# lmangani/duckdb-fastlane

Measured on AMD Instinct MI355X. Metric: decoded values/sec (lineitem_full SF100 full scan), higher is better.
Workload: dtype u8..u64 integer unpack -> int32/int64/string_t

## Files before the change

### duckdb-fastlane_amd/csrc/fls_decode.hpp

```cpp
#pragma once
#include <hip/hip_runtime.h>

#include <cstdint>
#include <vector>

namespace fls {

struct DevChunk {
    const uint8_t *chunk;
    const uint8_t *dict;
    uint8_t *out;
    uint32_t nvec;
    uint32_t dict_count;
    uint32_t meta_off;
    uint32_t packed_off;
    uint32_t aux_off;
    uint8_t enc, T, vbits, ob;
    uint64_t heap_host;
    uint32_t heap_bytes;
    union {
        uint32_t vec_base;
        uint32_t max_w;
    };
};
static_assert(sizeof(DevChunk) == 64, "DevChunk is 64 B");

enum : uint32_t { KERR_DICT_CODE = 1, KERR_RUN_INDEX = 2, KERR_BAD_DESC = 4, KERR_FSST = 8 };
enum : uint32_t { KERR_LDS_BASE = 32 };

struct DecodeGeom {
    uint32_t p_bytes = 256, v_bytes = 0;
    int grid = 0;
};

struct SplitPlan {
    uint32_t waves = 0, pieces = 0;
    bool guided = false;
    size_t positions() const { return waves ? (size_t)waves + pieces + 2 : 0; }
};

hipError_t launch_decode(const DevChunk *d_chunks, uint32_t nchunks, uint32_t *d_err, const DecodeGeom &geom,
                         hipStream_t stream, uint32_t *d_queue = nullptr, const uint32_t *d_split = nullptr,
                         SplitPlan plan = SplitPlan(), bool shared_queue = false, int prio = 0);
uint32_t decode_waves(const DecodeGeom &geom);
SplitPlan balanced_split(const DevChunk *h, uint32_t n, uint32_t nw, uint32_t static_pct, uint32_t pieces_per_wave,
                         std::vector<uint32_t> &pos);
SplitPlan guided_split(const DevChunk *h, uint32_t n, uint32_t nw, uint32_t factor, uint32_t min_vecs,
                       std::vector<uint32_t> &pos);
enum : int {
    kFsstPlain = 1, kFsstTwoQ = 2, kFsstZeroFlush = 4, kFsstW6 = 8, kFsstCirc = 16, kFsstLenFromSym = 32, kFsstAbsLds = 64, kFsstEarlyGather = 128,
    kFsstDefault = kFsstW6 | kFsstZeroFlush | kFsstAbsLds,
    kFsstSegSparse = kFsstPlain,
    kFsstSegPackedLen = kFsstLenFromSym,
    kFsstSegWide = kFsstCirc,
    kFsstSegDouble = kFsstEarlyGather,
    kFsstSegBatch = 256,
    kFsstAblateRecords = 512, kFsstAblateFlush = 1024, kFsstAblateWrite = 2048,
    kFsstSegLean = 4096,
    kFsstSegD8 = 8192,
    kFsstSegLazy = 16384,
    kFsstSegW4 = 32768
};
struct FsstLaunch {
    int bytes_per_lane = 8;
    bool small = false;
    uint32_t *queue = nullptr;
    bool reset_queue = true;
    int waves_per_cu = 0;
    int grid_cus = 0;
    int variant = kFsstDefault;
    bool seg = false;
    int seg_cap = 4096;
};
hipError_t launch_fsst(const DevChunk *d_chunks, uint32_t nchunks, uint32_t nvecs, uint32_t *d_err,
                       hipStream_t stream, const FsstLaunch &how);
struct FusedLaunch {
    uint32_t fsst_per16 = 6;
    uint32_t piece = 2;
    bool halving = false;
    uint32_t fsst_static_pct = 0;
    bool static_first = true;
    int waves_per_cu = 0;
    int x = 0;
    uint32_t tail_chunks = 0, tail_split = 1;
};
hipError_t launch_fused(const DevChunk *d_main, uint32_t nmain, const DevChunk *d_fsst, uint32_t nfsst,
                        uint32_t nfvecs, bool small, uint32_t *d_err, const DecodeGeom &geom, hipStream_t stream,
                        uint32_t *d_queues, const FusedLaunch &how);
bool fsst_variant_built(int variant, bool seg, int bytes_per_lane);
bool fused_x_built(int x);
hipError_t launch_fsst_sp(const DevChunk *d_chunks, uint32_t nchunks, uint32_t nvecs, uint32_t *d_err,
                          hipStream_t stream);
int decode_grid_size(uint32_t shmem_per_block);
int device_cus();
int occupancy(const void *kernel, int block, size_t shmem);

bool &rating_launch();

struct ProbeRegion {
    uint8_t *out;
    uint64_t bytes;
};
hipError_t probe_placement(const ProbeRegion *d_regions, uint32_t nregions, uint8_t *const *bufs,
                           const uint64_t *buf_bytes, uint32_t nbuf, int reps, hipStream_t stream, float *chunk_ms,
                           float *fill_ms);
inline void chunk_lds_need(uint8_t enc, uint8_t T, uint8_t ob, uint32_t dict_count, uint32_t max_w,
                           uint32_t &p_bytes, uint32_t &v_bytes) {
    p_bytes = 128 * max_w + 128;
    v_bytes = 0;
    if (enc == 2  && T < 64) v_bytes = 128 * T;
    if (enc == 4 ) v_bytes = 2048;
    if (enc == 3 ) {
        const uint32_t d = dict_count * ob;
        v_bytes = 4096 + (d <= 4096 ? ((d + 15) & ~15u) : 0);
    }
}

}
```

### duckdb-fastlane_amd/csrc/flsgpu.hip

```cpp
#include <fcntl.h>
#include <hip/hip_runtime.h>
#include <hip/hip_ext.h>
#include <sys/mman.h>
#include <sys/stat.h>
#include <unistd.h>

#include <algorithm>
#include <atomic>
#include <condition_variable>
#include <cstring>
#include <map>
#include <mutex>
#include <memory>
#include <string>
#include <chrono>
#include <cmath>
#include <thread>
#include <vector>

#include "../../include/flsgpu.h"
#include "fls_agg.hpp"
#include "fls_common.hpp"
#include "fls_config.hpp"
#include "fls_decode.hpp"
// ... 459 lines not shown
                }
        }
        auto d = std::make_unique<ScanDev>();
        d->dev = dev;
        return d;
    }
    void give(std::unique_ptr<ScanDev> d) {
        if (!d) return;
        d->sync();
        if (d->free_batches.size() != d->batches.size()) return;
        for (auto &sl : d->slots) {
            sl.busy = sl.starved = false;
            sl.hb = nullptr;
        }
        d->free_batches.clear();
        for (auto &b : d->batches) d->free_batches.push_back(b.get());
        std::lock_guard<std::mutex> lk(mu);
        size_t same = 0;
        for (auto &x : idle) same += x->dev == d->dev;
        if (same >= kIdlePerDev) return;
        const int dev = d->dev;
        idle.push_back(std::move(d));
        trim_locked(dev, idle_cap_bytes());
    }
    size_t idle_pinned() {
        std::lock_guard<std::mutex> lk(mu);
        size_t t = 0;
        for (auto &d : idle) t += pinned_bytes(*d);
        return t;
    }
};

}

struct fls_connection {
    std::vector<int> devices;
    std::shared_ptr<ConnRes> res = std::make_shared<ConnRes>();
};

struct SideStream {
    hipStream_t stream = nullptr;
    hipEvent_t fork = nullptr, join = nullptr;
    int cu_m = 0;
    hipStream_t cu_a = nullptr, cu_b = nullptr;
    hipEvent_t join_a = nullptr, join_b = nullptr;
    void release_cu() {
        for (hipStream_t *st : {&cu_a, &cu_b})
            if (*st) {
                hipStreamSynchronize(*st);
                hipStreamDestroy(*st);
                *st = nullptr;
            }
        for (hipEvent_t *e : {&join_a, &join_b})
            if (*e) {
                hipEventDestroy(*e);
                *e = nullptr;
            }
        cu_m = 0;
    }
};

namespace {

struct Resident {
    int dev = -1;
    uint32_t rg0 = 0, rg1 = 0;
    uint64_t base = 0;
    uint64_t first_row = 0, rows = 0;
    DevBuf<uint8_t> img;
    DevBuf<StrT> strtab;
    std::vector<uint64_t> strtab_off;
    DevBuf<uint32_t> err;
    DevBuf<uint32_t> queue;
    std::vector<DevBuf<uint8_t>> d_heap;
    std::vector<PinBuf<uint8_t>> h_heap;
    std::vector<uint64_t> heap_off;
    std::vector<DevBuf<uint8_t>> d_out;
    double placement_q = 0;
    float placement_ms = 0;
    DevBuf<DevChunk> d_chunks;
    std::vector<DevChunk> h_chunks;
    std::vector<uint8_t> mask;
    uint32_t nmain = 0;
    int64_t policy = -1;
    int64_t lpolicy = 0;
    FsstCounts fsst;
    SplitPlan split;
    ByteCount bytes;
    hipStream_t stream = nullptr;
    SideStream side;
    std::vector<hipEvent_t> ev_pool;
    uint32_t ev_used = 0;
    Resident() = default;
    Resident(const Resident &) = delete;
    Resident &operator=(const Resident &) = delete;
    ~Resident() {
        if (dev < 0) return;
        hipSetDevice(dev);
        if (stream) hipStreamSynchronize(stream);
        if (side.stream) hipStreamSynchronize(side.stream);
        if (stream) hipStreamDestroy(stream);
        if (side.stream) hipStreamDestroy(side.stream);
        if (side.fork) hipEventDestroy(side.fork);
        if (side.join) hipEventDestroy(side.join);
        side.release_cu();
        for (auto e : ev_pool) hipEventDestroy(e);
    }
};

}

struct DevImage {
    uint8_t *p = nullptr;
    int dev = -1;
    uint64_t lo = 0, hi = 0;
    std::unique_ptr<std::atomic<uint8_t>[]> present;
    uint32_t nrg = 0;
    ~DevImage() {
        if (p) {
            int cur = 0;
            hipGetDevice(&cur);
            hipSetDevice(dev);
            hipFree(p);
            hipSetDevice(cur);
        }
    }
};
void drop_file_images(const void *owner);
struct MappedFile {
    void *map = nullptr;
    size_t len = 0;
    FileMeta meta;
    ~MappedFile() {
        drop_file_images(this);
        if (map) munmap(map, len);
    }
};

struct ImageRegistry {
    std::mutex mu;
    ResidentSet<DevImage> set;
};
ImageRegistry &image_registry() {
    static auto *r = new ImageRegistry();
    return *r;
}
uint64_t resident_budget() {
    return (uint64_t)std::max<int64_t>(0, knob_value("FLS_SCAN_RESIDENT_MB")) << 20;
}
namespace {
uint64_t release_idle_images(int dev) {
    ImageRegistry &R = image_registry();
    ResidentSet<DevImage>::Evicted ev;
    std::lock_guard<std::mutex> lk(R.mu);
    const uint64_t b = R.set.release_idle(dev, ev);
    ev.clear();
    return b;
}
}
void drop_file_images(const void *owner) {
    ImageRegistry &R = image_registry();
    ResidentSet<DevImage>::Evicted ev;
    std::lock_guard<std::mutex> lk(R.mu);
    R.set.drop_owner(owner, ev);
    ev.clear();
}
// ... 64 lines not shown
                       uint8_t *d_out, ByteCount *bc, uint8_t *d_heap = nullptr, const uint8_t *h_heap = nullptr,
                       uint32_t code_w = 0, const uint8_t *d_ident = nullptr) {
    const ChunkRef &ch = t->meta.rgs[rg].chunks[col];
    const ChunkHeader &h = ch.hdr;
    DevChunk d;
    memset(&d, 0, sizeof(d));
    d.chunk = d_chunk;
    d.out = d_out;
    d.nvec = h.nvec;
    d.dict_count = h.dict_count;
    d.meta_off = (uint32_t)h.meta_off;
    d.packed_off = (uint32_t)h.packed_off;
    d.aux_off = (uint32_t)h.aux_off;
    d.enc = h.enc;
    d.T = h.T;
    d.vbits = h.vbits;
    d.ob = (uint8_t)out_bytes_of(t, col);
    if (h.enc == ENC_DICT) d.dict = h.is_str ? d_dict : d_chunk + h.aux_off;
    if (code_w && h.enc == ENC_DICT && h.is_str) {
        d.ob = (uint8_t)code_w;
        d.dict = code_w == 1 ? d_ident : d_ident + kIdent16;
    }
    bc->values += h.nvals;
    if (h.enc == ENC_FSST) {
        d.dict = d_heap;
        d.heap_host = (uint64_t)(uintptr_t)h_heap;
        d.heap_bytes = (uint32_t)h.reserved1;
        bc->out += (uint64_t)h.nvals * 16 + h.reserved1;
        bc->meta += 32ull * h.nvec + kFsstTableBytes;
        const uint8_t *meta = t->img + ch.off + h.meta_off;
        bool sp = true;
        for (uint32_t v = 0; v < h.nvec; ++v) {
            VecMeta vm;
            memcpy(&vm, meta + 32ull * v, 32);
            FsstVecHeader fh;
            memcpy(&fh, t->img + ch.off + h.aux_off + vm.aux_off, sizeof(fh));
            bc->packed += 128ull * vm.bw + 128ull * fh.clen_w + fh.comp_len;
            bc->meta += sizeof(fh);
            if (chunk_seg_codes(h) == kFsstSegCodes) bc->meta += sizeof(FsstSegHeader) + fsst_nseg(fh.comp_len);
            const uint64_t dmax = (uint64_t)vm.for_base + (vm.bw >= 32 ? 0xFFFFFFFFull : (1ull << vm.bw) - 1);
            const uint64_t cmax = (uint64_t)fh.clen_base + (fh.clen_w >= 32 ? 0xFFFFFFFFull : (1ull << fh.clen_w) - 1);
            if (vm.for_base < 0 || dmax > 255 || cmax > 255) sp = false;
        }
        const char *sg = getenv("FLS_FSST_SEG");
        bool short_syms = true;
        const uint8_t *lens = t->img + ch.off + h.aux_off + 8 * 256;
        for (uint32_t k = 0; k < h.dict_count && k < 255; ++k) short_syms &= lens[k] <= 7;
        const bool seg = chunk_seg_codes(h) == kFsstSegCodes && short_syms && !(sg && atoi(sg) == 0);
        d.vbits = (sp ? 1 : 0) | (seg ? 2 : 0);
        return d;
    }
    bc->out += (uint64_t)h.nvals * d.ob;
    bc->meta += 32ull * h.nvec;
    const uint8_t *meta = t->img + ch.off + h.meta_off;
    uint32_t max_w = 0;
    for (uint32_t v = 0; v < h.nvec; ++v) {
        VecMeta vm;
        memcpy(&vm, meta + 32ull * v, 32);
        bc->packed += 128ull * vm.bw;
        max_w = std::max<uint32_t>(max_w, vm.bw);
        if (h.enc == ENC_DELTA) bc->meta += 128;
        if (h.enc == ENC_RLE) bc->meta += 128 + (uint64_t)vm.aux_count * (h.vbits / 8);
        if (h.enc == ENC_ALP && alp_exceptions(vm.aux_count))
            bc->meta += alp_aux_bytes(alp_exceptions(vm.aux_count), h.vbits);
    }
    if (h.enc == ENC_DICT) bc->meta += (uint64_t)h.dict_count * (h.is_str ? d.ob : h.vbits / 8);
    d.max_w = max_w;
    uint32_t pb, vb;
    chunk_lds_need(h.enc, h.T, d.ob, h.dict_count, max_w, pb, vb);
    bc->geom.p_bytes = std::max(bc->geom.p_bytes, pb);
    bc->geom.v_bytes = std::max(bc->geom.v_bytes, vb);
    return d;
}

bool col_selected(const std::vector<uint8_t> &mask, uint32_t c) { return mask.empty() || mask[c]; }

bool is_fsst(const fls_table *t, uint32_t rg, uint32_t c) { return t->meta.rgs[rg].chunks[c].hdr.enc == ENC_FSST; }

enum : int {
    POLICY_STATIC = 1, POLICY_NO_LPT = 2, POLICY_FULL_PREFETCH = 4, POLICY_FSST_NOSEG = 8, POLICY_FSST16 = 16,
    POLICY_BALANCED = 32, POLICY_QUEUE = 64, POLICY_FSST_SP = 128
};
constexpr int kGuidedMinVecs = 0, kGuidedFactor = 2;
int64_t decode_policy() {
    const char *e = getenv("FLS_DECODE_POLICY");
    const char *sp = getenv("FLS_STATIC_PCT");
    const char *tp = getenv("FLS_TAIL_PIECES");
    const int pct = sp ? std::min(100, std::max(0, atoi(sp))) : 100;
    const int pieces = tp ? std::min(255, std::max(1, atoi(tp))) : 2;
    const char *bp = getenv("FLS_BLOCKS_PER_CU");
    const int bpc = bp ? std::min(127, std::max(0, atoi(bp))) : 0;
    const char *sg = getenv("FLS_FSST_SEG");
    const int noseg = sg && atoi(sg) == 0 ? POLICY_FSST_NOSEG : 0;
    const char *gm = getenv("FLS_GUIDED_MIN_VECS");
    const char *gf = getenv("FLS_GUIDED_FACTOR");
    const int64_t gmin = gm ? std::min(64, std::max(0, atoi(gm))) : kGuidedMinVecs;
    const int64_t gfac = gf ? std::min(255, std::max(1, atoi(gf))) : kGuidedFactor;
    return (int64_t)(((e ? (atoi(e) & 0xFF) : 0) | noseg) | pct << 8 | pieces << 16 | bpc << 24) | gmin << 32 |
           gfac << 40;
}

int64_t launch_policy(int64_t policy, const std::vector<DevChunk> &v, DecodeGeom &geom) {
    if (policy & (POLICY_STATIC | POLICY_BALANCED | POLICY_QUEUE)) return policy;
    size_t nmain = 0;
    for (const DevChunk &d : v) nmain += d.enc != ENC_FSST;
    if (geom.grid <= 0) geom.grid = decode_grid_size(4 * (geom.p_bytes + geom.v_bytes));
    return nmain < decode_waves(geom) ? (policy | POLICY_BALANCED) : policy;
}

uint32_t order_for_launch(std::vector<DevChunk> &v, FsstCounts *fc, int64_t policy) {
    auto mid = std::stable_partition(v.begin(), v.end(), [](const DevChunk &d) { return d.enc != ENC_FSST; });
    std::stable_sort(mid, v.end(), [](const DevChunk &a, const DevChunk &b) {
        return fsst_group(a.vbits) < fsst_group(b.vbits);
    });
    if (policy & POLICY_FULL_PREFETCH)
        for (auto it = v.begin(); it != mid; ++it) it->max_w = it->T;
    if (policy & POLICY_BALANCED) {
        std::stable_sort(v.begin(), mid, [](const DevChunk &a, const DevChunk &b) { return a.chunk < b.chunk; });
    } else if (!(policy & (POLICY_STATIC | POLICY_NO_LPT))) {
        std::stable_sort(v.begin(), mid, [](const DevChunk &a, const DevChunk &b) {
            return (uint64_t)a.nvec * a.ob > (uint64_t)b.nvec * b.ob;
        });
    }
    *fc = FsstCounts();
    for (auto it = mid; it != v.end(); ++it) {
        const int g = fsst_group(it->vbits);
        it->vec_base = fc->vecs[g];
        fc->vecs[g] += it->nvec;
        fc->n[g]++;
    }
    return (uint32_t)(mid - v.begin());
}

SplitPlan append_split(std::vector<DevChunk> &list, uint32_t nmain, const DecodeGeom &geom, int64_t policy) {
    if (nmain == 0) return SplitPlan();
    std::vector<uint32_t> pos;
    SplitPlan plan;
    if (policy & POLICY_BALANCED)
        plan = balanced_split(list.data(), nmain, decode_waves(geom), (policy >> 8) & 0xFF, (policy >> 16) & 0xFF, pos);
    else if (!(policy & (POLICY_STATIC | POLICY_NO_LPT)) && ((policy >> 32) & 0xFF))
        plan = guided_split(list.data(), nmain, decode_waves(geom), (uint32_t)((policy >> 40) & 0xFF),
                            (uint32_t)((policy >> 32) & 0xFF), pos);
    else
        return SplitPlan();
    const size_t k = list.size();
    list.resize(k + (pos.size() * 4 + sizeof(DevChunk) - 1) / sizeof(DevChunk));
    memcpy(list.data() + k, pos.data(), pos.size() * 4);
    return plan;
}

struct OverlapSplit {
    int decode_bpc = 1, fsst_wpc = 12;
    uint32_t min_vecs_per_cu = 800;
    int decode_prio = 0;
    int cu_split = 0;
    bool guided = false;
};
OverlapSplit overlap_split() {
    OverlapSplit o;
    if (const char *e = getenv("FLS_OVERLAP_CU_SPLIT")) o.cu_split = std::min(31, std::max(0, atoi(e)));
    if (const char *e = getenv("FLS_OVERLAP_DECODE_BPC")) o.decode_bpc = std::max(1, atoi(e));
    if (const char *e = getenv("FLS_OVERLAP_FSST_WPC")) o.fsst_wpc = std::max(0, atoi(e));
    if (const char *e = getenv("FLS_OVERLAP_MIN_VECS_PER_CU")) o.min_vecs_per_cu = (uint32_t)std::max(0, atoi(e));
    if (const char *e = getenv("FLS_OVERLAP_DECODE_PRIO")) o.decode_prio = std::min(3, std::max(0, atoi(e)));
    if (const char *e = getenv("FLS_OVERLAP_GUIDED")) o.guided = atoi(e) != 0;
    return o;
}

int fsst_config_check(int64_t policy) {
    int variant = kFsstDefault;
    const char *fv = getenv("FLS_FSST_VARIANT");
    if (fv) {
        char *end = nullptr;
        const long v = strtol(fv, &end, 10);
        if (end == fv || *end != 0 || v < 0 || v > 0x7FFFFFFF)
            return fail(FLS_ERR_CONFIG, "FLS_FSST_VARIANT=%s is not a variant number", fv);
        variant = (int)v;
    }
    if (const char *fx = getenv("FLS_FUSED_X")) {
        char *end = nullptr;
        const long x = strtol(fx, &end, 10);
        if (end == fx || *end != 0 || x < 0 || x > 0x7FFFFFFF || !fused_x_built((int)x))
            return fail(FLS_ERR_CONFIG,
                        "FLS_FUSED_X=%s is not in this build: the product library holds the default fused kernel "
                        "only; experiments need FLS_LIB=libflsgpu_lab.so (make lab) -- unset FLS_FUSED_X",
                        fx);
    }
    const int bpl = (policy & POLICY_FSST16) ? 16 : 8;
    if (!fsst_variant_built(variant, true, bpl) || !fsst_variant_built(variant, false, bpl))
        return fail(FLS_ERR_CONFIG,
                    "FSST kernel variant %d (%d bytes per lane) is not in this build: the product library holds the "
                    "default kernels only; experiments need FLS_LIB=libflsgpu_lab.so (make lab)%s",
                    variant, bpl, fv ? " -- unset FLS_FSST_VARIANT" : "");
// ... 12 lines not shown
FusedCfg fused_cfg() {
    FusedCfg f;
    if (const char *e = getenv("FLS_FUSED")) f.mode = std::min(2, std::max(0, atoi(e) == 1 ? 2 : atoi(e)));
    if (const char *e = getenv("FLS_FUSED_FSST16")) {
        f.how.fsst_per16 = (uint32_t)std::min(16, std::max(0, atoi(e)));
        f.per16_set = true;
    }
    if (const char *e = getenv("FLS_FUSED_PIECE")) f.how.piece = (uint32_t)std::min(64, std::max(1, atoi(e)));
    if (const char *e = getenv("FLS_FUSED_WPC")) f.how.waves_per_cu = std::max(0, atoi(e));
    if (const char *e = getenv("FLS_FUSED_STATIC_PCT")) f.how.fsst_static_pct = (uint32_t)std::min(100, std::max(0, atoi(e)));
    if (const char *e = getenv("FLS_FUSED_STATIC_FIRST")) f.how.static_first = atoi(e) != 0;
    if (const char *e = getenv("FLS_FUSED_HALVING")) f.how.halving = atoi(e) != 0;
    if (const char *e = getenv("FLS_FUSED_TAIL")) f.how.tail_chunks = (uint32_t)std::max(0, atoi(e));
    if (const char *e = getenv("FLS_FUSED_TAIL_SPLIT")) f.how.tail_split = (uint32_t)std::min(64, std::max(1, atoi(e)));
    if (const char *e = getenv("FLS_FUSED_X")) f.how.x = atoi(e);
    if (const char *e = getenv("FLS_FUSED_MIN_VECS_PER_CU")) f.min_vecs_per_cu = (uint32_t)std::max(0, atoi(e));
    if (const char *e = getenv("FLS_FSST_VARIANT"))
        if (atoi(e) != kFsstDefault) f.variant = true;
    return f;
}

template <class LaunchGroup>
hipError_t launch_cu_split(const DevChunk *d_chunks, uint32_t nmain, const FsstCounts &fc, uint32_t *d_err,
                           const DecodeGeom &geom, hipStream_t stream, uint32_t *d_queue, SideStream *side,
                           const OverlapSplit &ov, int cus, const FsstLaunch (&how)[kFsstGroups],
                           LaunchGroup &launch_group) {
    const int m = ov.cu_split;
    uint32_t mask_a[8] = {}, mask_b[8] = {};
    int na = 0, nb = 0;
    for (int i = 0; i < std::min(cus, 256); ++i) {
        if (i % 32 < m) {
            mask_a[i / 32] |= 1u << (i % 32);
            ++na;
        } else {
            mask_b[i / 32] |= 1u << (i % 32);
            ++nb;
        }
    }
    if (na == 0 || nb == 0) return hipErrorInvalidValue;
    if (side->cu_m != m) {
        side->release_cu();
        hipError_t e = hipExtStreamCreateWithCUMask(&side->cu_a, 8, mask_a);
        if (e == hipSuccess) e = hipExtStreamCreateWithCUMask(&side->cu_b, 8, mask_b);
        if (e == hipSuccess) e = hipEventCreateWithFlags(&side->join_a, hipEventDisableTiming);
        if (e == hipSuccess) e = hipEventCreateWithFlags(&side->join_b, hipEventDisableTiming);
        if (e != hipSuccess) {
            side->release_cu();
            return e;
        }
        side->cu_m = m;
    }
    const uint32_t shmem = 4 * (geom.p_bytes + geom.v_bytes);
    const int bpc = std::max(1, (geom.grid > 0 ? geom.grid : decode_grid_size(shmem)) / std::max(1, cus));
    DecodeGeom ga = geom, gb = geom;
    ga.grid = na * bpc;
    gb.grid = nb * bpc;
    FsstLaunch ha[kFsstGroups], hb[kFsstGroups];
    for (int g = 0; g < kFsstGroups; ++g) {
        ha[g] = hb[g] = how[g];
        ha[g].queue = hb[g].queue = d_queue + 1 + g;
        ha[g].reset_queue = hb[g].reset_queue = false;
        ha[g].grid_cus = na;
        hb[g].grid_cus = nb;
    }
    hipError_t e = hipMemsetAsync(d_queue, 0, kQueueWords * sizeof(uint32_t), stream);
    if (e == hipSuccess) e = hipEventRecord(side->fork, stream);
    if (e == hipSuccess) e = hipStreamWaitEvent(side->cu_a, side->fork, 0);
    if (e == hipSuccess) e = hipStreamWaitEvent(side->cu_b, side->fork, 0);
    if (e == hipSuccess)
        e = launch_decode(d_chunks, nmain, d_err, ga, side->cu_a, d_queue, nullptr, SplitPlan(), true, ov.decode_prio);
    for (int g = 0; g < kFsstGroups && e == hipSuccess; ++g) e = launch_group(g, side->cu_b, hb[g]);
    if (e == hipSuccess)
        e = launch_decode(d_chunks, nmain, d_err, gb, side->cu_b, d_queue, nullptr, SplitPlan(), true, ov.decode_prio);
    for (int g = 0; g < kFsstGroups && e == hipSuccess; ++g) e = launch_group(g, side->cu_a, ha[g]);
    if (e == hipSuccess) e = hipEventRecord(side->join_a, side->cu_a);
    if (e == hipSuccess) e = hipEventRecord(side->join_b, side->cu_b);
    if (e == hipSuccess) e = hipStreamWaitEvent(stream, side->join_a, 0);
    if (e == hipSuccess) e = hipStreamWaitEvent(stream, side->join_b, 0);
    return e;
}

hipError_t launch_all(const DevChunk *d_chunks, uint32_t nmain, uint32_t ntotal, const FsstCounts &fc,
                      uint32_t *d_err, const DecodeGeom &geom, hipStream_t stream, uint32_t *d_queue, int64_t policy,
                      SplitPlan plan, const SideStream *side = nullptr) {
    const uint32_t *d_split = plan.waves ? reinterpret_cast<const uint32_t *>(d_chunks + ntotal) : nullptr;
    const bool balanced = d_split && !plan.guided;
    const bool sp = (policy & POLICY_FSST_SP) != 0;
    const OverlapSplit ov = overlap_split();
    FsstLaunch how[kFsstGroups];
    for (int g = 0; g < kFsstGroups; ++g) {
        how[g].bytes_per_lane = (policy & POLICY_FSST16) ? 16 : 8;
        if (const char *fv = getenv("FLS_FSST_VARIANT")) how[g].variant = atoi(fv);
        how[g].small = g == 0 || g == 2;
        how[g].seg = g < 2;
        if (const char *sc = getenv("FLS_FSST_SEG_CAP")) how[g].seg_cap = atoi(sc);
    }
    auto launch_group = [&](int g, hipStream_t st, const FsstLaunch &h) -> hipError_t {
        const DevChunk *dc = d_chunks + nmain + fc.first(g);
        if (g == 2 && sp && !h.queue) return launch_fsst_sp(dc, fc.n[g], fc.vecs[g], d_err, st);
        return launch_fsst(dc, fc.n[g], fc.vecs[g], d_err, st, h);
    };
    const int cus = device_cus();
    const uint64_t fsst_vecs = fc.total_vecs();
    if (ov.cu_split > 0 && side && side->stream && nmain > 0 && fsst_vecs > 0 && !balanced && !sp &&
        !(policy & POLICY_STATIC))
        return launch_cu_split(d_chunks, nmain, fc, d_err, geom, stream, d_queue, const_cast<SideStream *>(side),
                               ov, cus, how, launch_group);
    {
        const FusedCfg fz = fused_cfg();
        int g1 = -1, ng = 0;
        for (int g = 0; g < kFsstGroups; ++g)
            if (fc.n[g]) {
                g1 = g;
                ++ng;
            }
        if (fz.mode > 0 && !fz.variant && ((ng == 1 && nmain > 0) || fz.mode == 2) && ng <= 1 && g1 < 2 && !balanced && !sp &&
            !(policy & POLICY_STATIC) &&
            fsst_vecs >= (uint64_t)fz.min_vecs_per_cu * (uint64_t)cus) {
            const int g = std::max(0, g1);
            FusedLaunch how = fz.how;
            if (!fz.per16_set) how.fsst_per16 = fsst_vecs < 1000ull * (uint64_t)cus ? 5u : 6u;
            return launch_fused(d_chunks, nmain, d_chunks + nmain + fc.first(g), fc.n[g], fc.vecs[g], g == 0, d_err,
                                geom, stream, d_queue, how);
        }
    }
    const bool overlap = side && side->stream && ov.fsst_wpc > 0 && nmain > 0 && fsst_vecs > 0 &&
                         fsst_vecs >= (uint64_t)ov.min_vecs_per_cu * (uint64_t)cus && !balanced && !sp &&
                         !(policy & POLICY_STATIC);
    hipError_t e = hipSuccess;
    if (overlap) {
        DecodeGeom narrow = geom;
        const uint32_t shmem = 4 * (geom.p_bytes + geom.v_bytes);
        narrow.grid = std::min(geom.grid > 0 ? geom.grid : decode_grid_size(shmem), cus * ov.decode_bpc);
        e = hipMemsetAsync(d_queue, 0, kQueueWords * sizeof(uint32_t), stream);
        if (e == hipSuccess) e = hipEventRecord(side->fork, stream);
        if (e == hipSuccess) e = hipStreamWaitEvent(side->stream, side->fork, 0);
        FsstLaunch narrow_how[kFsstGroups];
        for (int g = 0; g < kFsstGroups; ++g) {
            how[g].queue = d_queue + 1 + g;
            how[g].reset_queue = false;
            narrow_how[g] = how[g];
            narrow_how[g].waves_per_cu = ov.fsst_wpc;
        }
        const uint32_t *gs = d_split && plan.guided && ov.guided ? d_split : nullptr;
        const SplitPlan gp = gs ? plan : SplitPlan();
        if (e == hipSuccess)
            e = launch_decode(d_chunks, nmain, d_err, narrow, stream, d_queue, gs, gp, true, ov.decode_prio);
        for (int g = 0; g < kFsstGroups && e == hipSuccess; ++g) e = launch_group(g, side->stream, narrow_how[g]);
        if (e == hipSuccess)
            e = launch_decode(d_chunks, nmain, d_err, geom, side->stream, d_queue, gs, gp, true, ov.decode_prio);
        for (int g = 0; g < kFsstGroups && e == hipSuccess; ++g) e = launch_group(g, stream, how[g]);
        if (e == hipSuccess) e = hipEventRecord(side->join, side->stream);
        if (e == hipSuccess) e = hipStreamWaitEvent(stream, side->join, 0);
        return e;
    }
    e = launch_decode(d_chunks, nmain, d_err, geom, stream, (policy & POLICY_STATIC) ? nullptr : d_queue, d_split, plan);
    for (int g = 0; g < kFsstGroups && e == hipSuccess; ++g) e = launch_group(g, stream, how[g]);
    return e;
}

}

fls_table::~fls_table() {
    if (profiled && ScanProf::on()) scan_prof().print();
    resident.clear();
    for (ScanCtx *s : {&scan, &mat})
        for (auto &d : s->devs) {
            if (d) {
                d->sync();
                d->dimg.reset();
            }
            if (res) res->give(std::move(d));
            d.reset();
        }
    if (registered) hipHostUnregister((void *)img);
    if (map) munmap(map, map_len);
}


namespace {

bool term_may_match(const fls_table *t, uint32_t rg, const HostTerm &h) {
    const RowGroupMeta &r = t->meta.rgs[rg];
    const ChunkRef &ch = r.chunks[h.col];
    const bool all_null = !r.zones.empty() && (r.zones[h.col].flags & ZM_ALL_NULL);
    if (h.op == OP_FALSE) return false;
    if (h.op == OP_IS_NULL) return chunk_has_validity(ch.hdr);
    if (h.op == OP_IS_NOT_NULL) return !all_null;
    if (all_null) return false;
    if (h.kind == FK_STR) {
        if (ch.hdr.enc != ENC_DICT) return true;
        const uint8_t *aux = t->img + ch.off + ch.hdr.aux_off;
        for (uint32_t i = 0; i < ch.hdr.dict_count; ++i) {
            const uint8_t *p;
            uint32_t len;
            dict_string(aux, ch.hdr.dict_count, i, p, len);
            if (op_holds(h.op, cmp_bytes(p, len, (const uint8_t *)h.str.data(), (uint32_t)h.str.size())))
                return true;
        }
        return false;
    }
    if (r.zones.empty() || !(r.zones[h.col].flags & ZM_VALID)) return true;
    const ZoneMap &z = r.zones[h.col];
    int cmin, cmax;
// ... 1435 lines not shown
    return 0;
}

int fls_scan_dict_codes(fls_table *t, int enable) {
    if (!t) return fail(FLS_ERR_ARG, "fls_scan_dict_codes: NULL table");
    t->dict_codes = enable != 0;
    return 0;
}

int fls_table_validity(const fls_table *t, uint32_t rg, uint32_t col, const uint64_t **words) {
    if (!t || rg >= t->meta.rgs.size() || col >= t->meta.cols.size())
        return fail(FLS_ERR_ARG, "validity (%u, %u) out of range", rg, col);
    const uint64_t *w = chunk_validity_host(t, rg, col);
    if (words) *words = w;
    return w ? 1 : 0;
}

int fls_rowgroup_may_match(const fls_table *t, uint32_t rg, const fls_predicate *preds, uint32_t n) {
    if (!t || rg >= t->meta.rgs.size()) return fail(FLS_ERR_ARG, "row group %u out of range", rg);
    std::vector<HostTerm> terms;
    int rc = to_terms(t, preds, n, terms);
    if (rc) return rc;
    return rowgroup_may_match(t, rg, terms) ? 1 : 0;
}

int fls_scan_next(fls_table *t, fls_rowgroup *out) {
    if (!t || !out) return fail(FLS_ERR_ARG, "fls_scan_next: NULL argument");
    return scan_next(t, t->scan, out);
}

int fls_scan_acquire(fls_table *t, fls_rowgroup *out) {
    if (!t || !out) return fail(FLS_ERR_ARG, "fls_scan_acquire: NULL argument");
    return scan_acquire(t, t->scan, out);
}

int fls_scan_release(fls_table *t, uint32_t rowgroup) {
    if (!t) return fail(FLS_ERR_ARG, "fls_scan_release: NULL table");
    return scan_release(t, t->scan, rowgroup);
}


}

namespace {

int placement_tries() { return (int)std::max<int64_t>(1, knob_value("FLS_PLACEMENT_TRIES")); }

struct PlacementRating {
    float chunk_ms = 0, fill_ms = 0;
    double q = 0;
};

int rate_outputs(const fls_table *t, const Resident &r, const std::vector<DevBuf<uint8_t>> &outs,
                 PlacementRating &pr) {
    const uint32_t ncols = (uint32_t)t->meta.cols.size();
    std::vector<ProbeRegion> reg;
    for (uint32_t c = 0; c < ncols; ++c)
        for (uint32_t g = r.rg0; g < r.rg1; ++g) {
            const uint64_t ob = out_bytes_of(t, c);
            const uint64_t bytes = (t->meta.rgs[g].nrows * ob) & ~1023ull;
            if (bytes) reg.push_back({outs[c].p + (t->meta.rgs[g].first_row - r.first_row) * ob, bytes});
        }
    std::stable_sort(reg.begin(), reg.end(), [](const ProbeRegion &a, const ProbeRegion &b) { return a.bytes > b.bytes; });
    DevBuf<ProbeRegion> d;
    HIP_TRY(d.alloc(r.dev, reg.size()));
    HIP_TRY(hipMemcpy(d.p, reg.data(), reg.size() * sizeof(ProbeRegion), hipMemcpyHostToDevice));
    std::vector<uint8_t *> bufs(ncols);
    std::vector<uint64_t> sizes(ncols);
    for (uint32_t c = 0; c < ncols; ++c) {
        bufs[c] = outs[c].p;
        sizes[c] = (r.rows * out_bytes_of(t, c)) & ~4095ull;
    }
    HIP_TRY(probe_placement(d.p, (uint32_t)reg.size(), bufs.data(), sizes.data(), ncols, 2, r.stream, &pr.chunk_ms,
                            &pr.fill_ms));
    pr.q = pr.chunk_ms > 0 ? pr.fill_ms / pr.chunk_ms : 0;
    return 0;
}

int decode_part(fls_table *t, Resident &r, const std::vector<uint8_t> &mask);

float decode_rating(fls_table *t, Resident &r) {
    const uint32_t ncols = (uint32_t)t->meta.cols.size();
    const std::vector<uint8_t> mask(ncols, 1);
    r.h_chunks.clear();
    const uint32_t ev0 = r.ev_used;
    struct RatingScope {
        RatingScope() { rating_launch() = true; }
        ~RatingScope() { rating_launch() = false; }
    } scope;
    constexpr int kWarm = 2, kTimed = 3;
    bool ok = true;
    for (int i = 0; i < kWarm + kTimed && ok; ++i) ok = decode_part(t, r, mask) == 0;
    ok = ok && hipStreamSynchronize(r.stream) == hipSuccess;
    float ms = -1;
    for (int i = kWarm; i < kWarm + kTimed && ok; ++i) {
        float x = 0;
        ok = hipEventElapsedTime(&x, r.ev_pool[ev0 + 2 * i], r.ev_pool[ev0 + 2 * i + 1]) == hipSuccess;
        if (ok && (ms < 0 || x < ms)) ms = x;
    }
    uint32_t e = 0;
    ok = ok && hipMemcpy(&e, r.err.p, sizeof(e), hipMemcpyDeviceToHost) == hipSuccess && e == 0;
    (void)hipGetLastError();
    (void)hipMemset(r.err.p, 0, sizeof(uint32_t));
    r.ev_used = ev0;
    r.h_chunks.clear();
    return ok ? ms : -1.0f;
}

struct Candidate {
    std::vector<DevBuf<uint8_t>> out, heap;
    DevBuf<uint8_t> img;
    void clear() {
        out.clear();
        heap.clear();
        img.release();
    }
    void swap_into(Resident &r) {
        std::swap(r.d_out, out);
        if (!heap.empty()) std::swap(r.d_heap, heap);
        if (img.p) {
            std::swap(r.img.p, img.p);
            std::swap(r.img.n, img.n);
            std::swap(r.img.dev, img.dev);
        }
    }
};
bool placement_flag(const char *name) { return knob_value(name) != 0; }

bool alloc_candidate(const fls_table *t, const Resident &r, uint64_t set_bytes, Candidate &cand) {
    const uint32_t ncols = (uint32_t)t->meta.cols.size();
    const bool heaps = placement_flag("FLS_PLACEMENT_HEAPS"), image = placement_flag("FLS_PLACEMENT_IMAGE");
    uint64_t extra = image ? r.img.n : 0;
    for (uint32_t c = 0; heaps && c < ncols; ++c) extra += r.d_heap[c].p ? r.d_heap[c].n : 0;
    size_t fr = 0, tot = 0;
    if (hipMemGetInfo(&fr, &tot) != hipSuccess || fr < set_bytes + extra + (set_bytes + extra) / 8 + (1ull << 30)) {
        (void)hipGetLastError();
        return false;
    }
    cand.clear();
    auto make = [&](DevBuf<uint8_t> &b, size_t n) {
        if (hipMalloc((void **)&b.p, std::max<size_t>(1, n)) != hipSuccess) {
            (void)hipGetLastError();
            b.p = nullptr;
            return false;
        }
        b.n = n;
        b.dev = r.dev;
        return true;
    };
    cand.out.resize(ncols);
    bool ok = true;
    for (uint32_t c = 0; c < ncols && ok; ++c) ok = make(cand.out[c], r.rows * out_bytes_of(t, c));
    if (ok && heaps) {
        cand.heap.resize(ncols);
        for (uint32_t c = 0; c < ncols && ok; ++c)
            if (r.d_heap[c].p) ok = make(cand.heap[c], r.d_heap[c].n);
    }
    if (ok && image) ok = make(cand.img, r.img.n) && hipMemcpy(cand.img.p, r.img.p, r.img.n, hipMemcpyDeviceToDevice) == hipSuccess;
    if (!ok) {
        (void)hipGetLastError();
        cand.clear();
    }
    return ok;
}

int choose_placement(fls_table *t, Resident &r) {
    const uint32_t ncols = (uint32_t)t->meta.cols.size();
    uint64_t set_bytes = 0;
    for (uint32_t c = 0; c < ncols; ++c) set_bytes += r.rows * out_bytes_of(t, c);
    if (set_bytes < (256ull << 20)) return 0;
    const bool dbg = getenv("FLS_DEBUG") != nullptr;
    const int ndec = (int)std::max<int64_t>(0, knob_value("FLS_PLACEMENT_DECODE"));
    float best_ms = ndec > 1 ? decode_rating(t, r) : -1.0f;
    if (best_ms > 0) {
        if (dbg) fprintf(stderr, "DEBUG: placement dev %d set 0: decode %.3f ms\n", r.dev, best_ms);
        int kept = 0;
        Candidate cand;
        for (int k = 1; k < ndec && alloc_candidate(t, r, set_bytes, cand); ++k) {
            cand.swap_into(r);
            const float ms = decode_rating(t, r);
            if (dbg) fprintf(stderr, "DEBUG: placement dev %d set %d: decode %.3f ms\n", r.dev, k, ms);
            if (ms > 0 && ms < best_ms) {
                best_ms = ms;
                kept = k;
            } else {
                cand.swap_into(r);
            }
            cand.clear();
        }
        r.placement_ms = best_ms;
        if (dbg) fprintf(stderr, "DEBUG: placement dev %d kept set %d (decode %.3f ms)\n", r.dev, kept, best_ms);
        return 0;
    }
    const int tries = placement_tries();
    if (tries <= 1) return 0;
    const double good = knob_value("FLS_PLACEMENT_GOOD") / 1000.0;
    PlacementRating best;
    if (const int rc = rate_outputs(t, r, r.d_out, best)) return rc;
    if (dbg)
        fprintf(stderr, "DEBUG: placement dev %d set 0: chunk order %.3f ms, fill %.3f ms, q %.3f\n", r.dev,
                best.chunk_ms, best.fill_ms, best.q);
    int kept = 0;
    Candidate cand;
    for (int k = 1; k < tries && best.q < good && alloc_candidate(t, r, set_bytes, cand); ++k) {
        PlacementRating pr;
        if (const int rc = rate_outputs(t, r, cand.out, pr)) return rc;
        if (dbg)
            fprintf(stderr, "DEBUG: placement dev %d set %d: chunk order %.3f ms, fill %.3f ms, q %.3f\n", r.dev, k,
                    pr.chunk_ms, pr.fill_ms, pr.q);
        if (pr.q > best.q) {
            cand.swap_into(r);
            best = pr;
            kept = k;
        }
        cand.clear();
    }
    r.placement_q = best.q;
    if (dbg) fprintf(stderr, "DEBUG: placement dev %d kept set %d (q %.3f)\n", r.dev, kept, best.q);
    return 0;
}

int upload_part(fls_table *t, Resident &r) {
    HIP_TRY(hipSetDevice(r.dev));
    if (!r.stream) HIP_TRY(hipStreamCreateWithFlags(&r.stream, hipStreamNonBlocking));
    uint64_t lo, hi;
    rg_byte_range(t->meta, r.rg0, r.rg1, lo, hi);
    r.base = lo;
    HIP_TRY(r.img.alloc(r.dev, hi - lo + kImagePad));
    HIP_TRY(hipMemcpy(r.img.p, t->img + lo, hi - lo, hipMemcpyHostToDevice));
    std::vector<StrT> host;
    int rc = build_strtabs(t, r.dev, r.rg0, r.rg1, r.strtab, r.strtab_off, host);
    if (rc) return rc;
    HIP_TRY(r.err.alloc(r.dev, 1));
    HIP_TRY(hipMemset(r.err.p, 0, sizeof(uint32_t)));
    const uint32_t ncols = (uint32_t)t->meta.cols.size();
    r.first_row = t->meta.rgs[r.rg0].first_row;
    r.rows = t->meta.rgs[r.rg1 - 1].first_row + t->meta.rgs[r.rg1 - 1].nrows - r.first_row;
    r.d_out.resize(ncols);
    for (uint32_t c = 0; c < ncols; ++c) HIP_TRY(r.d_out[c].alloc(r.dev, r.rows * out_bytes_of(t, c)));
    r.heap_off.assign((size_t)(r.rg1 - r.rg0) * ncols, 0);
    r.d_heap.resize(ncols);
    r.h_heap.resize(ncols);
    for (uint32_t c = 0; c < ncols; ++c) {
        uint64_t tot = 0;
        for (uint32_t g = r.rg0; g < r.rg1; ++g) {
            r.heap_off[(size_t)(g - r.rg0) * ncols + c] = tot;
            if (is_fsst(t, g, c)) tot += t->meta.rgs[g].chunks[c].hdr.reserved1;
        }
        if (tot) {
            HIP_TRY(r.d_heap[c].alloc(r.dev, tot));
            HIP_TRY(r.h_heap[c].alloc(tot));
        } else {
            r.d_heap[c].release();
            r.h_heap[c].release();
        }
    }
    r.h_chunks.clear();
    r.mask.clear();
    if (const int prc = choose_placement(t, r)) return prc;
    if (getenv("FLS_DEBUG")) {
        fprintf(stderr, "DEBUG: part dev %d rg [%u, %u) image %p %llu B\n", r.dev, r.rg0, r.rg1, (void *)r.img.p,
                (unsigned long long)(hi - lo));
        for (uint32_t c = 0; c < ncols; ++c)
            fprintf(stderr, "DEBUG:   col %u out %p %llu B heap %p\n", c, (void *)r.d_out[c].p,
                    (unsigned long long)(r.rows * out_bytes_of(t, c)), (void *)r.d_heap[c].p);
    }
    return 0;
}

int decode_part(fls_table *t, Resident &r, const std::vector<uint8_t> &mask) {
    const uint32_t ncols = (uint32_t)t->meta.cols.size();
    HIP_TRY(hipSetDevice(r.dev));
    const int64_t policy = decode_policy();
    if (mask != r.mask || r.h_chunks.empty() || policy != r.policy) {
        std::vector<DevChunk> chunks;
        ByteCount bc;
        for (uint32_t c = 0; c < ncols; ++c) {
            if (!mask[c]) continue;
            for (uint32_t g = r.rg0; g < r.rg1; ++g) {
                const ChunkRef &ch = t->meta.rgs[g].chunks[c];
                const uint64_t so = r.strtab_off[(size_t)(g - r.rg0) * ncols + c];
                const uint8_t *dict = so == UINT64_MAX ? nullptr : (const uint8_t *)(r.strtab.p + so);
                uint8_t *out = r.d_out[c].p + (t->meta.rgs[g].first_row - r.first_row) * out_bytes_of(t, c);
                const uint64_t ho = r.heap_off[(size_t)(g - r.rg0) * ncols + c];
                chunks.push_back(make_devchunk(t, g, c, r.img.p + (ch.off - r.base), dict, out, &bc,
                                               r.d_heap[c].p ? r.d_heap[c].p + ho : nullptr,
                                               r.h_heap[c].p ? r.h_heap[c].p + ho : nullptr));
            }
        }
        const int64_t lpol = launch_policy(policy, chunks, bc.geom);
        r.nmain = order_for_launch(chunks, &r.fsst, lpol);
        r.policy = policy;
        r.lpolicy = lpol;
        const size_t k = chunks.size();
        r.split = append_split(chunks, r.nmain, bc.geom, lpol);
        HIP_TRY(hipStreamSynchronize(r.stream));
        HIP_TRY(r.d_chunks.alloc(r.dev, chunks.size()));
        HIP_TRY(hipMemcpy(r.d_chunks.p, chunks.data(), chunks.size() * sizeof(DevChunk), hipMemcpyHostToDevice));
        chunks.resize(k);
        r.h_chunks.swap(chunks);
        r.mask = mask;
        r.bytes = bc;
    }
    if (r.ev_used + 2 > r.ev_pool.size()) {
        for (int i = 0; i < 2; ++i) {
            hipEvent_t e;
            HIP_TRY(hipEventCreate(&e));
            r.ev_pool.push_back(e);
        }
    }
    HIP_TRY(r.queue.alloc(r.dev, kQueueWords));
    if (!r.side.stream) {
        HIP_TRY(hipStreamCreateWithFlags(&r.side.stream, hipStreamNonBlocking));
        HIP_TRY(hipEventCreateWithFlags(&r.side.fork, hipEventDisableTiming));
        HIP_TRY(hipEventCreateWithFlags(&r.side.join, hipEventDisableTiming));
    }
    if (r.fsst.total_vecs() > 0)
        if (const int rc = fsst_config_check(r.lpolicy)) return rc;
    hipEvent_t e0 = r.ev_pool[r.ev_used], e1 = r.ev_pool[r.ev_used + 1];
    r.ev_used += 2;
    HIP_TRY(hipEventRecord(e0, r.stream));
    HIP_TRY(launch_all(r.d_chunks.p, r.nmain, (uint32_t)r.h_chunks.size(), r.fsst, r.err.p, r.bytes.geom, r.stream,
                       r.queue.p, r.lpolicy, r.split, &r.side));
    HIP_TRY(hipEventRecord(e1, r.stream));
    return 0;
}

uint64_t resident_rows(const fls_table *t) {
    uint64_t n = 0;
    for (auto &r : t->resident) n += r->rows;
    return n;
}

const Resident *part_of(const fls_table *t, uint32_t part) {
    return t && part < t->resident.size() ? t->resident[part].get() : nullptr;
}

}

extern "C" {

int fls_device_upload(fls_table *t, uint32_t rg_begin, uint32_t rg_end) {
    if (!t) return fail(FLS_ERR_ARG, "fls_device_upload: NULL table");
    if (rg_end > t->meta.rgs.size() || rg_begin >= rg_end)
        return fail(FLS_ERR_ARG, "row-group range [%u,%u) out of bounds", rg_begin, rg_end);
    const uint32_t G = (uint32_t)t->devices.size(), n = rg_end - rg_begin;
    t->resident.clear();
    t->launches = 0;
    for (uint32_t g = 0; g < G; ++g) {
        const uint32_t a = rg_begin + (uint32_t)((uint64_t)n * g / G), b = rg_begin + (uint32_t)((uint64_t)n * (g + 1) / G);
        if (a == b) continue;
        auto r = std::make_unique<Resident>();
        r->dev = t->devices[g];
        r->rg0 = a;
        r->rg1 = b;
        int rc = upload_part(t, *r);
        t->resident.push_back(std::move(r));
        if (rc) {
            t->resident.clear();
            return rc;
        }
    }
    return 0;
}

int fls_device_decode(fls_table *t, const uint8_t *col_mask) {
    if (!t) return fail(FLS_ERR_ARG, "fls_device_decode: NULL table");
    if (t->resident.empty()) return fail(FLS_ERR_STATE, "fls_device_decode before fls_device_upload");
    const uint32_t ncols = (uint32_t)t->meta.cols.size();
    std::vector<uint8_t> mask(ncols, 1);
    if (col_mask)
        for (uint32_t c = 0; c < ncols; ++c) mask[c] = col_mask[c] ? 1 : 0;
    for (auto &r : t->resident) {
        int rc = decode_part(t, *r, mask);
        if (rc) return rc;
    }
    t->launches++;
    return 0;
}

int fls_device_sync(fls_table *t, fls_decode_stats *stats) {
    if (!t) return fail(FLS_ERR_ARG, "fls_device_sync: NULL table");
    if (t->resident.empty()) return fail(FLS_ERR_STATE, "nothing uploaded");
    uint32_t err = 0;
    for (auto &r : t->resident) {
        HIP_TRY(hipSetDevice(r->dev));
        HIP_TRY(hipStreamSynchronize(r->stream));
        uint32_t e = 0;
        HIP_TRY(hipMemcpy(&e, r->err.p, sizeof(e), hipMemcpyDeviceToHost));
        err |= e;
    }
    if (stats) {
        memset(stats, 0, sizeof(*stats));
        const uint32_t nl = t->resident[0]->ev_used / 2;
        double total = 0, last = 0;
        for (uint32_t i = 0; i < nl; ++i) {
            double span = 0;
            for (auto &r : t->resident) {
                if (2 * i + 1 >= r->ev_used) continue;
                float ms = 0;
                HIP_TRY(hipSetDevice(r->dev));
                HIP_TRY(hipEventElapsedTime(&ms, r->ev_pool[2 * i], r->ev_pool[2 * i + 1]));
                span = std::max(span, (double)ms);
            }
            total += span;
            last = span;
// ... 91 lines not shown
```

Before: 453.5 billion.

## Route small-dictionary VARCHAR chunks to a dedicated per-vector workgroup kernel

Adds a specialized kernel that decodes 32-bit dictionary-coded 16-byte string columns with small dictionaries (up to 64 entries). It uses one 256-thread block per vector, stages the dictionary in LDS and writes with vectorized 16-byte stores. The host pulls eligible chunks out of the main decode list, interleaves them across output streams, and builds a per-vector descriptor list that is launched before the main decode. The aim is to take skewed dictionary-string work off the generic decoder and raise memory parallelism. The cost is an extra kernel launch, a per-vector descriptor array, and a change to the fused FSST split ratio when this path is active.

After: 472.8 billion (median of 6 runs). +4.2%, better.

```diff
diff --git a/duckdb-fastlane_amd/csrc/fls_decode.hpp b/duckdb-fastlane_amd/csrc/fls_decode.hpp
--- a/duckdb-fastlane_amd/csrc/fls_decode.hpp
+++ b/duckdb-fastlane_amd/csrc/fls_decode.hpp
@@ -91,6 +91,21 @@
 bool fused_x_built(int x);
 hipError_t launch_fsst_sp(const DevChunk *d_chunks, uint32_t nchunks, uint32_t nvecs, uint32_t *d_err,
                           hipStream_t stream);
+struct DictVec {
+    const uint8_t *packed;
+    const uint8_t *tab;
+    uint8_t *out;
+    uint32_t base;
+    uint32_t info;
+};
+static_assert(sizeof(DictVec) == 32, "DictVec is 32 B");
+constexpr uint32_t kDictWgMaxEntries = 64;
+inline bool dictstr_eligible(const DevChunk &c) {
+    return c.enc == 3  && c.ob == 16 && c.T == 32 && c.nvec > 0 && c.dict_count >= 1 &&
+           c.dict_count <= kDictWgMaxEntries && c.dict && ((uintptr_t)c.dict & 15) == 0 && ((uintptr_t)c.out & 15) == 0 &&
+           (((uintptr_t)c.chunk + c.packed_off) & 15) == 0;
+}
+hipError_t launch_dictstr(const DictVec *d_vecs, uint32_t nvecs, uint32_t *d_err, hipStream_t stream);
 int decode_grid_size(uint32_t shmem_per_block);
 int device_cus();
 int occupancy(const void *kernel, int block, size_t shmem);
diff --git a/duckdb-fastlane_amd/csrc/fls_dictstr.hip b/duckdb-fastlane_amd/csrc/fls_dictstr.hip
--- /dev/null
+++ b/duckdb-fastlane_amd/csrc/fls_dictstr.hip
@@ -0,0 +1,86 @@
+#include <hip/hip_runtime.h>
+
+#include <cstdio>
+#include <cstdlib>
+
+#include "fls_decode.hpp"
+#include "fls_format.hpp"
+#include "fls_unpack.hpp"
+
+namespace fls {
+using namespace dev;
+namespace {
+
+constexpr uint32_t kRounds = kVectorSize / 256;
+static_assert(kDictWgMaxEntries == 64, "one wave stages the table, one entry per lane");
+
+}
+
+template <bool RATING>
+__global__ __launch_bounds__(256) void dictstr_decode_kernel(const DictVec *__restrict__ vecs,
+                                                             uint32_t *__restrict__ err) {
+    __shared__ v4u tab[kDictWgMaxEntries];
+    typedef uint32_t v8u __attribute__((ext_vector_type(8)));
+    const v8u q = ((const __attribute__((address_space(4))) v8u *)vecs)[blockIdx.x];
+    const uint64_t packed = (uint64_t)q[1] << 32 | q[0], tab_g = (uint64_t)q[3] << 32 | q[2];
+    const uint64_t out_g = (uint64_t)q[5] << 32 | q[4];
+    const uint32_t base = q[6], info = q[7];
+    const uint32_t t = threadIdx.x;
+    const uint32_t nvals = info & 2047u, W = (info >> 11) & 63u, n = info >> 17;
+    const bool stager = uni(t >> 6) == 0;
+    v4u te = mk4(0, 0, 0, 0);
+    if (stager) te = ((const FLS_GLOBAL v4u *)tab_g)[min(t, n - 1)];
+    uint32_t code[kRounds];
+    if (W == 0) {
+#pragma unroll
+        for (uint32_t r = 0; r < kRounds; ++r) code[r] = 0;
+    } else {
+        const FLS_GLOBAL uint32_t *pk = ((const FLS_GLOBAL uint32_t *)packed) + (t & 31);
+        const uint32_t mask = W >= 32 ? 0xFFFFFFFFu : (1u << W) - 1u;
+        uint32_t lo[kRounds], hi[kRounds];
+#pragma unroll
+        for (uint32_t r = 0; r < kRounds; ++r) {
+            const uint32_t k = ((8 * r + (t >> 5)) * W) >> 5;
+            lo[r] = pk[32 * k];
+            hi[r] = pk[32 * min(k + 1, W - 1)];
+        }
+#pragma unroll
+        for (uint32_t r = 0; r < kRounds; ++r)
+            code[r] = __builtin_amdgcn_alignbit(hi[r], lo[r], ((8 * r + (t >> 5)) * W) & 31) & mask;
+    }
+    if (stager) tab[t] = te;
+    bool bad = false;
+#pragma unroll
+    for (uint32_t r = 0; r < kRounds; ++r) {
+        code[r] += base;
+        if (code[r] >= n) {
+            bad = true;
+            code[r] = n - 1;
+        }
+    }
+    __syncthreads();
+    v4u e[kRounds];
+#pragma unroll
+    for (uint32_t r = 0; r < kRounds; ++r) e[r] = tab[code[r]];
+    FLS_GLOBAL v4u *out = ((FLS_GLOBAL v4u *)out_g) + t;
+    if (nvals == kVectorSize) {
+#pragma unroll
+        for (uint32_t r = 0; r < kRounds; ++r) out[256 * r] = e[r];
+    } else {
+#pragma unroll
+        for (uint32_t r = 0; r < kRounds; ++r)
+            if (256 * r + t < nvals) out[256 * r] = e[r];
+    }
+    if (__any(bad) && (t & 63) == 0) atomicOr(err, KERR_DICT_CODE);
+}
+
+hipError_t launch_dictstr(const DictVec *d_vecs, uint32_t nvecs, uint32_t *d_err, hipStream_t stream) {
+    if (nvecs == 0) return hipSuccess;
+    auto kern = rating_launch() ? dictstr_decode_kernel<true> : dictstr_decode_kernel<false>;
+    if (getenv("FLS_DEBUG"))
+        fprintf(stderr, "DEBUG: dictstr_decode_kernel: %u blocks of 256 threads, %u vectors\n", nvecs, nvecs);
+    hipLaunchKernelGGL(kern, dim3(nvecs), dim3(256), 0, stream, d_vecs, d_err);
+    return hipGetLastError();
+}
+
+}
diff --git a/duckdb-fastlane_amd/csrc/flsgpu.hip b/duckdb-fastlane_amd/csrc/flsgpu.hip
--- a/duckdb-fastlane_amd/csrc/flsgpu.hip
+++ b/duckdb-fastlane_amd/csrc/flsgpu.hip
@@ -565,6 +565,14 @@
     std::vector<DevChunk> h_chunks;
     std::vector<uint8_t> mask;
     uint32_t nmain = 0;
+    DevBuf<DictVec> d_dictvecs;
+    uint32_t ndictvecs = 0;
+    bool list_built = false;
+    void invalidate() {
+        h_chunks.clear();
+        ndictvecs = 0;
+        list_built = false;
+    }
     int64_t policy = -1;
     int64_t lpolicy = 0;
     FsstCounts fsst;
@@ -795,6 +803,18 @@
     POLICY_BALANCED = 32, POLICY_QUEUE = 64, POLICY_FSST_SP = 128
 };
 constexpr int kGuidedMinVecs = 0, kGuidedFactor = 2;
+struct DictWgCfg {
+    int mode = 1;
+    uint32_t min_vecs_per_cu = 64;
+    uint32_t streams = 4;
+};
+DictWgCfg dict_wg_cfg() {
+    DictWgCfg c;
+    if (const char *e = getenv("FLS_DICT_WG")) c.mode = std::min(2, std::max(0, atoi(e)));
+    if (const char *e = getenv("FLS_DICT_WG_MIN_VECS_PER_CU")) c.min_vecs_per_cu = (uint32_t)std::min(255, std::max(0, atoi(e)));
+    if (const char *e = getenv("FLS_DICT_WG_STREAMS")) c.streams = (uint32_t)std::min(31, std::max(1, atoi(e)));
+    return c;
+}
 int64_t decode_policy() {
     const char *e = getenv("FLS_DECODE_POLICY");
     const char *sp = getenv("FLS_STATIC_PCT");
@@ -809,8 +829,9 @@
     const char *gf = getenv("FLS_GUIDED_FACTOR");
     const int64_t gmin = gm ? std::min(64, std::max(0, atoi(gm))) : kGuidedMinVecs;
     const int64_t gfac = gf ? std::min(255, std::max(1, atoi(gf))) : kGuidedFactor;
+    const DictWgCfg dw = dict_wg_cfg();
     return (int64_t)(((e ? (atoi(e) & 0xFF) : 0) | noseg) | pct << 8 | pieces << 16 | bpc << 24) | gmin << 32 |
-           gfac << 40;
+           gfac << 40 | (int64_t)dw.mode << 48 | (int64_t)dw.min_vecs_per_cu << 50 | (int64_t)dw.streams << 58;
 }
 
 int64_t launch_policy(int64_t policy, const std::vector<DevChunk> &v, DecodeGeom &geom) {
@@ -821,7 +842,32 @@
     return nmain < decode_waves(geom) ? (policy | POLICY_BALANCED) : policy;
 }
 
-uint32_t order_for_launch(std::vector<DevChunk> &v, FsstCounts *fc, int64_t policy) {
+uint32_t order_for_launch(std::vector<DevChunk> &v, FsstCounts *fc, int64_t policy,
+                          std::vector<DevChunk> *dictwg = nullptr) {
+    if (dictwg) {
+        dictwg->clear();
+        const int mode = (int)((policy >> 48) & 3);
+        uint64_t vecs = 0;
+        for (const DevChunk &d : v)
+            if (dictstr_eligible(d)) vecs += d.nvec;
+        const uint64_t need = mode == 2 ? 1 : (uint64_t)((policy >> 50) & 0xFF) * (uint64_t)device_cus();
+        if (mode > 0 && vecs > 0 && vecs >= need && vecs <= UINT32_MAX) {
+            auto rest = std::stable_partition(v.begin(), v.end(), [](const DevChunk &d) { return !dictstr_eligible(d); });
+            dictwg->assign(rest, v.end());
+            v.erase(rest, v.end());
+            std::stable_sort(dictwg->begin(), dictwg->end(),
+                             [](const DevChunk &a, const DevChunk &b) { return a.out < b.out; });
+            const size_t n = dictwg->size(), S = std::min<size_t>(std::max<size_t>(1, (size_t)((policy >> 58) & 31)), n);
+            if (S > 1) {
+                std::vector<DevChunk> il;
+                il.reserve(n);
+                for (size_t i = 0; il.size() < n; ++i)
+                    for (size_t s = 0; s < S; ++s)
+                        if (s * n / S + i < (s + 1) * n / S) il.push_back((*dictwg)[s * n / S + i]);
+                dictwg->swap(il);
+            }
+        }
+    }
     auto mid = std::stable_partition(v.begin(), v.end(), [](const DevChunk &d) { return d.enc != ENC_FSST; });
     std::stable_sort(mid, v.end(), [](const DevChunk &a, const DevChunk &b) {
         return fsst_group(a.vbits) < fsst_group(b.vbits);
@@ -1000,7 +1046,12 @@
 
 hipError_t launch_all(const DevChunk *d_chunks, uint32_t nmain, uint32_t ntotal, const FsstCounts &fc,
                       uint32_t *d_err, const DecodeGeom &geom, hipStream_t stream, uint32_t *d_queue, int64_t policy,
-                      SplitPlan plan, const SideStream *side = nullptr) {
+                      SplitPlan plan, const SideStream *side = nullptr, const DictVec *d_dictvecs = nullptr,
+                      uint32_t ndictvecs = 0) {
+    if (ndictvecs) {
+        const hipError_t de = launch_dictstr(d_dictvecs, ndictvecs, d_err, stream);
+        if (de != hipSuccess || ntotal == 0) return de;
+    }
     const uint32_t *d_split = plan.waves ? reinterpret_cast<const uint32_t *>(d_chunks + ntotal) : nullptr;
     const bool balanced = d_split && !plan.guided;
     const bool sp = (policy & POLICY_FSST_SP) != 0;
@@ -1037,7 +1088,7 @@
             fsst_vecs >= (uint64_t)fz.min_vecs_per_cu * (uint64_t)cus) {
             const int g = std::max(0, g1);
             FusedLaunch how = fz.how;
-            if (!fz.per16_set) how.fsst_per16 = fsst_vecs < 1000ull * (uint64_t)cus ? 5u : 6u;
+            if (!fz.per16_set) how.fsst_per16 = ndictvecs ? 8u : fsst_vecs < 1000ull * (uint64_t)cus ? 5u : 6u;
             return launch_fused(d_chunks, nmain, d_chunks + nmain + fc.first(g), fc.n[g], fc.vecs[g], g == 0, d_err,
                                 geom, stream, d_queue, how);
         }
@@ -2639,7 +2690,7 @@
 float decode_rating(fls_table *t, Resident &r) {
     const uint32_t ncols = (uint32_t)t->meta.cols.size();
     const std::vector<uint8_t> mask(ncols, 1);
-    r.h_chunks.clear();
+    r.invalidate();
     const uint32_t ev0 = r.ev_used;
     struct RatingScope {
         RatingScope() { rating_launch() = true; }
@@ -2660,7 +2711,7 @@
     (void)hipGetLastError();
     (void)hipMemset(r.err.p, 0, sizeof(uint32_t));
     r.ev_used = ev0;
-    r.h_chunks.clear();
+    r.invalidate();
     return ok ? ms : -1.0f;
 }
 
@@ -2812,7 +2863,7 @@
             r.h_heap[c].release();
         }
     }
-    r.h_chunks.clear();
+    r.invalidate();
     r.mask.clear();
     if (const int prc = choose_placement(t, r)) return prc;
     if (getenv("FLS_DEBUG")) {
@@ -2829,7 +2880,7 @@
     const uint32_t ncols = (uint32_t)t->meta.cols.size();
     HIP_TRY(hipSetDevice(r.dev));
     const int64_t policy = decode_policy();
-    if (mask != r.mask || r.h_chunks.empty() || policy != r.policy) {
+    if (mask != r.mask || !r.list_built || policy != r.policy) {
         std::vector<DevChunk> chunks;
         ByteCount bc;
         for (uint32_t c = 0; c < ncols; ++c) {
@@ -2846,7 +2897,25 @@
             }
         }
         const int64_t lpol = launch_policy(policy, chunks, bc.geom);
-        r.nmain = order_for_launch(chunks, &r.fsst, lpol);
+        std::vector<DevChunk> dictwg;
+        r.nmain = order_for_launch(chunks, &r.fsst, lpol, &dictwg);
+        std::vector<DictVec> dvecs;
+        for (const DevChunk &d : dictwg) {
+            const uint8_t *meta = t->img + r.base + (d.chunk - r.img.p) + d.meta_off;
+            for (uint32_t v = 0; v < d.nvec; ++v) {
+                VecMeta vm;
+                memcpy(&vm, meta + 32ull * v, 32);
+                dvecs.push_back(DictVec{d.chunk + d.packed_off + vm.packed_off, d.dict,
+                                        d.out + (size_t)v * kVectorSize * 16, (uint32_t)vm.for_base,
+                                        (uint32_t)vm.nvals | (uint32_t)vm.bw << 11 | d.dict_count << 17});
+            }
+        }
+        if (getenv("FLS_DEBUG")) {
+            size_t kept = 0;
+            for (size_t i = 0; i < r.nmain; ++i) kept += chunks[i].enc == ENC_DICT && chunks[i].ob == 16;
+            fprintf(stderr, "DEBUG: dictstr_decode_kernel takes %zu chunks (%zu vectors), %zu DICT VARCHAR chunks stay "
+                            "on the main decode\n", dictwg.size(), dvecs.size(), kept);
+        }
         r.policy = policy;
         r.lpolicy = lpol;
         const size_t k = chunks.size();
@@ -2854,6 +2923,11 @@
         HIP_TRY(hipStreamSynchronize(r.stream));
         HIP_TRY(r.d_chunks.alloc(r.dev, chunks.size()));
         HIP_TRY(hipMemcpy(r.d_chunks.p, chunks.data(), chunks.size() * sizeof(DevChunk), hipMemcpyHostToDevice));
+        HIP_TRY(r.d_dictvecs.alloc(r.dev, dvecs.size()));
+        if (!dvecs.empty())
+            HIP_TRY(hipMemcpy(r.d_dictvecs.p, dvecs.data(), dvecs.size() * sizeof(DictVec), hipMemcpyHostToDevice));
+        r.ndictvecs = (uint32_t)dvecs.size();
+        r.list_built = true;
         chunks.resize(k);
         r.h_chunks.swap(chunks);
         r.mask = mask;
@@ -2878,7 +2952,7 @@
     r.ev_used += 2;
     HIP_TRY(hipEventRecord(e0, r.stream));
     HIP_TRY(launch_all(r.d_chunks.p, r.nmain, (uint32_t)r.h_chunks.size(), r.fsst, r.err.p, r.bytes.geom, r.stream,
-                       r.queue.p, r.lpolicy, r.split, &r.side));
+                       r.queue.p, r.lpolicy, r.split, &r.side, r.d_dictvecs.p, r.ndictvecs));
     HIP_TRY(hipEventRecord(e1, r.stream));
     return 0;
 }
```
